# kevinh-e/BetaOne

Measured on AMD Instinct MI355X. Metric: mcts_nodes_per_sec, higher is better.
Workload: dtype f32 (3 x f16 split, f32 accumulate)

## Files before the change

betaone_amd/csrc/bo_chess.h:

```cpp
#pragma once
#include "bo_wave.h"

#define BO_MAX_MOVES 256
#define BO_NUM_ACTIONS 4672

enum { BB_P = 0, BB_N = 1, BB_B = 2, BB_R = 3, BB_Q = 4, BB_K = 5, BB_WHITE = 6, BB_BLACK = 7 };

struct DPos {
    uint64_t bb[8];
    uint32_t flags;
    int32_t halfmove;
    int32_t fullmove;
    uint32_t khash;
};
#define F_TURN 0x1u
#define F_CASTLE_SHIFT 1
#define F_CASTLE_MASK 0x1Eu
#define F_EP_SHIFT 8
#define F_EP_MASK (0x7Fu << 8)
#define F_IRREV 0x8000u
#define F_EPKEY_SHIFT 16
#define F_EPKEY_MASK (0x7Fu << 16)
#define F_KEY_MASK (F_TURN | F_CASTLE_MASK | F_EPKEY_MASK)

// ... 358 lines not shown
    o = bC + ((i1 >> 16) & 255) - cC;
    for (uint64_t t = tC; t;) {
        int to = bo_msb64(t);
        t ^= BIT(to);
        if (BIT(to) & promo_rank) { out[o++] = MV(s, to, 5); out[o++] = MV(s, to, 4); out[o++] = MV(s, to, 3); out[o++] = MV(s, to, 2); }
        else out[o++] = MV(s, to, 0);
    }
    o = b1 + ((i1 >> 24) & 255) - c1;
    if (t1) {
        int to = bo_lsb64(t1);
        if (t1 & promo_rank) { out[o++] = MV(s, to, 5); out[o++] = MV(s, to, 4); out[o++] = MV(s, to, 3); out[o++] = MV(s, to, 2); }
        else out[o++] = MV(s, to, 0);
    }
    if (t2) out[b2 + (i2 & 255) - c2] = MV(s, bo_lsb64(t2), 0);
    if (epc) out[bF + ((i2 >> 8) & 255) - cF] = MV(s, pos_ep(P), 0);
    bo_sync();
    *in_check_out = nchk > 0;
    return total;
}
BO_DEV_NOINLINE int bo_movegen(const DPos &P, bo_mv *out, bool *in_check_out) { return bo_movegen_inline(P, out, in_check_out); }
```

betaone_amd/csrc/bo_engine.cpp:

```cpp
#include "../../include/betaone_engine.h"
#include "../../include/betaone_lab.h"

#include "bo_tree.h"
#include "bo_fastw.h"
#include "bo_select_wide.h"
#include "bo_replay.h"
#include "bo_train.h"
#include "bo_pgn.h"
#include "bo_san.h"
#include "bo_analyse.h"
#include "bo_perft.h"
#include "bo_nn_fused.h"
#include "bo_conv.h"
#include "bo_tower.h"
#include "bo_tower_wg.h"
#include "bo_tower_h.h"
#include "bo_tower_s.h"
#include "bo_tower_s16.h"
#include "bo_tower_h16.h"
#include "bo_heads.h"
#include "bo_tower_b1.h"
#include "bo_rt.h"
#include "bo_hostrng.h"

// ... 16 lines not shown
        int _rc = (call);                                                                            \
        if (_rc != 0) return fail(BO_E_HIP, std::string(#call) + ": " + rt_errstr(_rc));             \
    } while (0)

struct bo_engine {
    Eng d;
    FastW f;
    int fast_reuse = 1;
    int sel_profile = 0, sel_pending = 0;
    long long sel_launches = 0;
    double sel_ms = 0.0;
#if !defined(BO_WAVE_EMU)
    hipEvent_t sel_ev0 = nullptr, sel_ev1 = nullptr;
#endif
    bool fast = false;
    bo_config cfg;
    int device;
    std::vector<void *> allocs;
    int *d_go = nullptr, *d_action = nullptr;
    std::vector<int> h_i32;
    std::vector<HostRng> rng;
    int *d_res_blk = nullptr, *d_info_blk = nullptr;
    int *h_res = nullptr, *h_info = nullptr;
    int watch_seen = 0;
    double *h_noise = nullptr;
    int *h_go = nullptr;
    int *h_action = nullptr;
    int action_flip = 0;
    rt_event ev_action[2]{};
    bool ev_action_made[2] = {false, false};
// ... 157 lines not shown
    for (int k = 1; k <= cfg->mcts_batch_size; k++) {
        const double r = (double)(int)(cfg->widen_coeff * sqrt((double)k)) / (double)k;
        if (r > per_sim) per_sim = r;
    }
    c.NCAP = fast ? 2 : (int)ceil(c.S * per_sim) + 2 * root_m + 4;
    c.nstride = c.NCAP;
    c.PLY_CAP = cfg->max_plies; c.TRK_CAP = cfg->max_plies;
    c.UL_MAX = fast ? 1 : c.B; c.CH_MAX = ch_max < 1 ? 1 : ch_max;
    c.cpuct = (float)cfg->cpuct;
    c.keep = (float)(1.0 - cfg->dirichlet_epsilon);
    c.eps = cfg->dirichlet_epsilon;
    c.use_noise = cfg->dirichlet_alpha > 0 ? 1 : 0;
    c.root_m = root_m;
    c.profile = 0;
    { const char *v = getenv("BETAONE_BURST_TWO_PATHS"); c.burst_two = (v && v[0] == '0') ? 0 : 1; }
    c.root_q = 0;
    const size_t G = (size_t)c.G, N = G * (size_t)c.NCAP;
    Eng &d = e->d;
    int rc = 0;
    float *sq = nullptr, *rcp = nullptr; int *wl = nullptr;
    rc |= e->alloc(&sq, (size_t)c.S + 2); rc |= e->alloc(&wl, (size_t)c.B + 1); rc |= e->alloc(&rcp, (size_t)c.S + 3);
    int **iscal[] = {&d.sims_done, &d.n_nodes, &d.rows, &d.n_runs, &d.n_ul, &d.req_nlegal, &d.status,
                     &d.trk_n, &d.n_hist, &d.ctx_mode, &d.root_nch, &d.stat_evals,
                     &d.stat_flushes, &d.stat_term_sims, &d.stat_levels, &d.stat_children_scanned, &e->d_go, &e->d_action};
    for (int **p : iscal) rc |= e->alloc(p, G);
    const size_t res_ints = G * (4 + 2 * (size_t)BO_RES_CAP) + 4, info_ints = G * 18;
    rc |= e->alloc(&e->d_res_blk, res_ints); rc |= e->alloc(&e->d_info_blk, info_ints);
    if (!rc) {
        d.res_n = e->d_res_blk; d.res_best_idx = e->d_res_blk + G; d.res_best_mv = e->d_res_blk + 2 * G; d.res_total = e->d_res_blk + 3 * G;
        d.res_idx = e->d_res_blk + 4 * G; d.res_val = reinterpret_cast<float *>(e->d_res_blk + 4 * G + G * BO_RES_CAP);
        d.res_watch = e->d_res_blk + G * (4 + 2 * (size_t)BO_RES_CAP); d.watch = nullptr; d.watch_n = 1;
        d.phase = e->d_info_blk; d.req_node = e->d_info_blk + G; d.root_nlegal = e->d_info_blk + 2 * G; d.root_term = e->d_info_blk + 3 * G;
        d.ply = e->d_info_blk + 4 * G;
        e->d_turn_action = e->d_info_blk + 5 * G; e->d_turn_state = e->d_info_blk + 6 * G; e->d_turn_cres = e->d_info_blk + 7 * G;
        e->d_turn_rv = reinterpret_cast<float *>(e->d_info_blk + 15 * G); e->d_turn_resigned = e->d_info_blk + 16 * G;
        e->d_turn_rnext = e->d_info_blk + 17 * G;
        rt_memset(e->d_res_blk, 0, res_ints * 4, nullptr); rt_memset(e->d_info_blk, 0, info_ints * 4, nullptr);
    }
    rc |= rt_host_alloc((void **)&e->h_res, res_ints * 4); rc |= rt_host_alloc((void **)&e->h_info, info_ints * 4);
    rc |= rt_host_alloc((void **)&e->h_noise, G * BO_MAX_MOVES * sizeof(double)); rc |= rt_host_alloc((void **)&e->h_go, G * 4);
    rc |= rt_host_alloc((void **)&e->h_action, 2 * G * 4);
    rc |= rt_host_alloc((void **)&e->h_turn_u, G * sizeof(double)); rc |= rt_host_alloc((void **)&e->h_turn_flags, G * 4);
    rc |= e->alloc(&e->d_turn_pw, (size_t)cfg->num_simulations + 1);
    { const char *v = getenv("BETAONE_TURN_COPIES"); e->ship = !(v && v[0] == '1'); }
    rc |= e->alloc(&d.gpos, G * c.PLY_CAP); rc |= e->alloc(&d.trk, G * c.TRK_CAP); rc |= e->alloc(&d.trk_cnt, G * c.TRK_CAP);
    rc |= e->alloc(&d.hist, G * 7);
    rc |= e->alloc(&d.n_visits, N); rc |= e->alloc(&d.parent, N); rc |= e->alloc(&d.first_child, N); rc |= e->alloc(&d.n_children, N);
    rc |= e->alloc(&d.q, N); rc |= e->alloc(&d.prior, N); rc |= e->alloc(&d.move, N); rc |= e->alloc(&d.term, N);
    rc |= e->alloc(&d.eval_slot, N); rc |= e->alloc(&d.npos, N);
    rc |= e->alloc(&d.run_leaf, G * c.B); rc |= e->alloc(&d.run_cnt, G * c.B);
    rc |= e->alloc(&d.ul_node, G * c.UL_MAX); rc |= e->alloc(&d.ul_nlegal, G * c.UL_MAX); rc |= e->alloc(&d.ul_value, G * c.UL_MAX);
    rc |= e->alloc(&d.ul_move, G * c.UL_MAX * BO_CH_CAP); rc |= e->alloc(&d.ul_prior, G * c.UL_MAX * BO_CH_CAP);
    rc |= e->alloc(&d.req_moves, G * BO_MAX_MOVES); rc |= e->alloc(&d.root_moves, G * BO_MAX_MOVES);
    rc |= e->alloc(&d.root_child_rank, G * 2 * BO_CH_CAP); rc |= e->alloc(&d.noise, G * BO_MAX_MOVES);
    rc |= e->alloc(&d.played, G * c.PLY_CAP);
    rc |= e->alloc(&d.prof, G * BO_PROF_SLOTS);
    rc |= e->alloc(&d.resign_cnt, 2 * G); rc |= e->alloc(&e->d_root_value, G);
    if (!rc) rt_memset(d.resign_cnt, 0, 2 * G * 4, nullptr);
    d.played_now = nullptr;
    if (fast) {
        FastW &f = e->f;
        const size_t L = (size_t)cfg->leaves_per_step;
        f.L = (int)L;
        f.sel_ut = 2; f.sel_flags = FW_SEL_OCT;
        const size_t expansions = (size_t)c.S + L + 2;
        f.NG = cfg->fast_arena_granules > 0 ? cfg->fast_arena_granules : (int)((6 * expansions + 8) * (32 / BO_FW_GR));
        if (f.NG < 64 || f.NG > BO_FW_LINK_MASK) { bo_engine_destroy(e); return fail(BO_E_ARG, "fast_arena_granules out of range (64 .. 2^24 - 1)"); }
        const size_t NR = (size_t)f.NG * BO_FW_GR;
        rc |= e->alloc(&f.arena, G * 2 * NR); rc |= e->alloc(&f.amove, G * 2 * NR);
        f.CS = (FWC_HEAD + FWR_FIELDS * (int)L + 31) / 32 * 32;
        rc |= e->alloc(&f.ctl, G * (size_t)f.CS);
// ... 248 lines not shown
            if (e->sel_pending) {
                float ms = 0.0f;
                RT((int)hipEventSynchronize(e->sel_ev1));
                RT((int)hipEventElapsedTime(&ms, e->sel_ev0, e->sel_ev1));
                e->sel_ms += ms; e->sel_launches++; e->sel_pending = 0;
            }
            RT((int)hipEventRecord(e->sel_ev0, (hipStream_t)stream));
        }
#endif
        RT(launch_fw_select(e, value_dev, policy_kind, stream));
#if !defined(BO_WAVE_EMU)
        if (e->sel_profile) { RT((int)hipEventRecord(e->sel_ev1, (hipStream_t)stream)); e->sel_pending = 1; }
#endif
        RT(RT_LAUNCH(bo_k_fw_leaf, rows, stream, e->d, e->f, nn_in_dev));
    } else {
        RT(RT_LAUNCH(bo_k_step, e->d.c.G, stream, e->d, policy_dev, value_dev, policy_kind, nn_in_dev, vt));
    }
    return BO_OK;
}
extern "C" int bo_step(bo_engine *e, const float *policy_dev, const float *value_dev, int policy_kind, float *nn_in_dev,
                       void *stream) {
    if (!e || !nn_in_dev) return fail(BO_E_ARG, "null argument");
    if (policy_kind != BO_POLICY_NONE && (!policy_dev || !value_dev)) return fail(BO_E_ARG, "policy/value required");
    return step_launch(e, policy_dev, value_dev, policy_kind, nn_in_dev, stream, StepTail{nullptr, nullptr, nullptr, nullptr, 0});
}
extern "C" int bo_step_heads(bo_engine *e, const float *logits_dev, const float *vpart_dev, const float *b1_dev, const float *w2_dev,
                             const float *b2_dev, int rows, float *nn_in_dev, void *stream) {
    if (!e || !nn_in_dev || !logits_dev || !vpart_dev || !b1_dev || !w2_dev || !b2_dev) return fail(BO_E_ARG, "null argument");
    if (e->fast) return fail(BO_E_CONFIG, "bo_step_heads: the reference-semantics search only (fast mode evaluates rows, not games)");
    if (rows < e->d.c.G) return fail(BO_E_ARG, "bo_step_heads: the partial sums must hold a row per game (rows >= G)");
    return step_launch(e, logits_dev, nullptr, BO_POLICY_LOGITS, nn_in_dev, stream, StepTail{vpart_dev, b1_dev, w2_dev, b2_dev, rows});
// ... 2185 lines not shown
```

betaone_amd/csrc/bo_rt.h:

```cpp
#pragma once
#include <stddef.h>
#include <stdlib.h>
#include <string.h>

#if defined(BO_WAVE_EMU)
static inline int rt_set_device(int) { return 0; }
static inline int rt_malloc(void **p, size_t n) { *p = malloc(n ? n : 1); if (*p) memset(*p, 0xCD, n); return *p ? 0 : -1; }
static inline void rt_free(void *p) { free(p); }
static inline int rt_h2d(void *d, const void *h, size_t n, void *) { memcpy(d, h, n); return 0; }
static inline int rt_d2h(void *h, const void *d, size_t n, void *) { memcpy(h, d, n); return 0; }
static inline int rt_memset(void *d, int v, size_t n, void *) { memset(d, v, n); return 0; }
static inline int rt_sync(void *) { return 0; }
static inline int rt_host_alloc(void **p, size_t n) { *p = calloc(n ? n : 1, 1); return *p ? 0 : -1; }
static inline void rt_host_free(void *p) { free(p); }
static inline int rt_h2d_2d(void *d, size_t dpitch, const void *h, size_t hpitch, size_t width, size_t height, void *) {
    for (size_t r = 0; r < height; r++) memcpy((char *)d + r * dpitch, (const char *)h + r * hpitch, width);
    return 0;
}
static inline int rt_d2h_2d(void *h, size_t hpitch, const void *d, size_t dpitch, size_t width, size_t height, void *) {
    for (size_t r = 0; r < height; r++) memcpy((char *)h + r * hpitch, (const char *)d + r * dpitch, width);
    return 0;
}
typedef int rt_event;
static inline int rt_event_create(rt_event *) { return 0; }
static inline int rt_event_record(rt_event, void *) { return 0; }
static inline int rt_event_sync(rt_event) { return 0; }
static inline void rt_event_destroy(rt_event) {}
static inline const char *rt_errstr(int) { return "emulator error"; }
#define RT_LAUNCH(kernel, grid, stream, ...) (bo_emu::launch((grid), [&]() { kernel(__VA_ARGS__); }), 0)
#else
#include <hip/hip_runtime.h>
static inline int rt_set_device(int d) { return (int)hipSetDevice(d); }
static inline int rt_malloc(void **p, size_t n) { return (int)hipMalloc(p, n ? n : 1); }
static inline void rt_free(void *p) { (void)hipFree(p); }
static inline int rt_h2d(void *d, const void *h, size_t n, void *s) { return (int)hipMemcpyAsync(d, h, n, hipMemcpyHostToDevice, (hipStream_t)s); }
static inline int rt_d2h(void *h, const void *d, size_t n, void *s) { return (int)hipMemcpyAsync(h, d, n, hipMemcpyDeviceToHost, (hipStream_t)s); }
static inline int rt_memset(void *d, int v, size_t n, void *s) { return (int)hipMemsetAsync(d, v, n, (hipStream_t)s); }
static inline int rt_sync(void *s) { return (int)hipStreamSynchronize((hipStream_t)s); }
static inline int rt_host_alloc(void **p, size_t n) { return (int)hipHostMalloc(p, n ? n : 1, hipHostMallocDefault); }
static inline void rt_host_free(void *p) { (void)hipHostFree(p); }
static inline int rt_h2d_2d(void *d, size_t dpitch, const void *h, size_t hpitch, size_t width, size_t height, void *s) {
    return (int)hipMemcpy2DAsync(d, dpitch, h, hpitch, width, height, hipMemcpyHostToDevice, (hipStream_t)s);
}
static inline int rt_d2h_2d(void *h, size_t hpitch, const void *d, size_t dpitch, size_t width, size_t height, void *s) {
    return (int)hipMemcpy2DAsync(h, hpitch, d, dpitch, width, height, hipMemcpyDeviceToHost, (hipStream_t)s);
}
typedef hipEvent_t rt_event;
static inline int rt_event_create(rt_event *ev) { return (int)hipEventCreateWithFlags(ev, hipEventDisableTiming); }
static inline int rt_event_record(rt_event ev, void *s) { return (int)hipEventRecord(ev, (hipStream_t)s); }
static inline int rt_event_sync(rt_event ev) { return (int)hipEventSynchronize(ev); }
static inline void rt_event_destroy(rt_event ev) { (void)hipEventDestroy(ev); }
static inline const char *rt_errstr(int e) { return hipGetErrorString((hipError_t)e); }
#define RT_LAUNCH(kernel, grid, stream, ...)                                                                   \
    ([&]() -> int {                                                                                            \
        hipLaunchKernelGGL(kernel, dim3((unsigned)(grid)), dim3(64), 0, (hipStream_t)(stream), __VA_ARGS__);   \
        return (int)hipGetLastError();                                                                         \
    }())
#endif
```

betaone_amd/csrc/bo_tree.h:

```cpp
#pragma once
#include "bo_chess.h"
#include <math.h>

#define BO_CH_CAP 32
#define BO_PATH_CAP 1024
#define BO_RES_CAP 256
#define BO_PLANES 120
#ifndef BO_PROF_SLOTS
#define BO_PROF_SLOTS 16
#endif
#define BO_ROW (BO_PLANES * 64)

enum { PH_IDLE = 0, PH_RUN = 1, PH_DONE = 2 };
enum { ST_OK = 0, ST_NODE_OVERFLOW = 1, ST_DEPTH_OVERFLOW = 2, ST_NAN_SCORE = 4, ST_PLY_OVERFLOW = 8,
       ST_ILLEGAL_ACTION = 16, ST_UL_OVERFLOW = 32, ST_TRK_OVERFLOW = 64 };
enum { POLICY_NONE = 0, POLICY_LOGITS = 1, POLICY_PROBS = 2 };

struct EngCfg {
    int G, S, B;
    int NCAP, PLY_CAP, TRK_CAP;
    int nstride;
    int UL_MAX, CH_MAX;
    float cpuct, keep;
    double eps;
    int use_noise;
    int root_m;
    int profile;
    int burst_two;
    int root_q;
};

struct Eng {
    EngCfg c;
    const float *sqrt_lut;
    const float *rcp_lut;
    const int *widen_lut;
    int *phase, *sims_done, *n_nodes, *rows, *n_runs, *n_ul, *req_node, *req_nlegal, *status;
    int *ply, *trk_n, *n_hist, *ctx_mode, *root_nlegal, *root_term, *root_nch;
    int *stat_evals, *stat_flushes, *stat_term_sims, *stat_levels, *stat_children_scanned;
    DPos *gpos, *trk, *hist;
    int *trk_cnt;
    int *n_visits, *parent, *first_child, *n_children;
    float *q, *prior;
// ... 4 lines not shown
    int *run_leaf, *run_cnt;
    int *ul_node, *ul_nlegal;
    float *ul_value;
    bo_mv *ul_move;
    float *ul_prior;
    bo_mv *req_moves, *root_moves;
    int *root_child_rank;
    double *noise;
    bo_mv *played;
    int *res_n, *res_idx, *res_best_idx, *res_best_mv, *res_total;
    float *res_val;
    int watch_n;
    int *watch, *res_watch;
    int *played_now;
    int *resign_cnt;
    unsigned long long *prof;
};

#define NOFF(e, g) ((size_t)(g) * (size_t)(e).c.nstride)

BO_DEV float bo_expf(float x) {
#if defined(BO_WAVE_EMU)
    return expf(x);
#else
    return __expf(x);
#endif
}
struct bo_f4 { float x, y, z, w; };
BO_DEV float bo_exp_row(float x) { return expf(x); }
#if defined(BO_WAVE_EMU)
// ... 84 lines not shown
        const int node = in ? path[j] : 0;
        const uint32_t fl = in ? e.npos[no + node].flags : 0u;
        const uint32_t kh = in ? e.npos[no + node].khash : 0u;
        const uint64_t irr = bo_ballot(in && j >= 1 && (fl & F_IRREV));
        const uint64_t below = BIT(lane) - 1;
        const bool take = in && j < d && (irr & below) == 0;
        const uint64_t tk = bo_ballot(take);
        if (take) {
            const int o = cnt + bo_popc64(tk & below);
            if (o < BO_CHAIN_CAP) { cb.hash[o] = kh; cb.ref[o] = node; }
        }
        cnt += bo_popc64(tk);
        stop = irr != 0;
    }
    if (!stop) cnt = chain_collect_history(e, g, cb, cnt);
    bo_sync();
    return cnt;
}

template <class PosFn, class CollectFn>
BO_DEV int terminal_eval_with(const Eng &e, int g, PosFn tree_pos, const DPos &P, const bo_mv *mv, int n, bool in_check, bo_mv *scratch,
                              ChainBuf &cb, CollectFn collect) {
    if (n == 0 && in_check) return 1;
    if (insufficient_material(P)) return 2;
    if (n == 0) return 2;
    if (P.halfmove >= 150) return 2;
    const int npred = collect();
    const int nn = npred < BO_CHAIN_CAP ? npred : BO_CHAIN_CAP;
    int same = 0;
    for (int i = bo_lane(); i < nn; i += 64)
        if (cb.hash[i] == P.khash && key_equal(chain_entry(e, g, tree_pos, cb.ref[i]), P)) same++;
// ... 72 lines not shown
BO_DEV void encode_static(const Eng &e, int g, float *row) {
    const int s = bo_lane();
    const int nh = e.n_hist[g];
    const DPos *h = e.hist + (size_t)g * 7;
    for (int pl = 0; pl < (7 - nh) * 14; pl++) row[pl * 64 + s] = 0.0f;
    for (int i = 0; i < nh; i++) {
        DPos H = h[i];
        encode_block(row, 7 - nh + i, H, tracker_reps(e, g, H));
    }
}
BO_DEV void encode_leaf(const Eng &e, int g, float *row, const DPos &P) {
    encode_block(row, 7, P, tracker_reps(e, g, P));
    encode_scalars(row, P);
}

BO_DEV int select_leaf(const Eng &e, int g, int *flags, int *path, int *depth_out, const float *lut) {
    const size_t no = NOFF(e, g);
    const int lane = bo_lane();
    int cur = 0, levels = 0, scanned = 0;
    if (lane == 0) path[0] = 0;
    int nc = e.n_children[no], fc = e.first_child[no];
    int pv = e.n_visits[no], pv_next = pv;
    for (;;) {
        if (nc == 0) break;
        const float sp = lut[pv];
        float score = -__builtin_inff();
        int n = 0, c_fc = 0, c_nc = 0;
        if (lane < nc) {
            n = e.n_visits[no + fc + lane];
            c_fc = e.first_child[no + fc + lane];
            c_nc = e.n_children[no + fc + lane];
// ... 28 lines not shown
        score = __builtin_bit_cast(float, bo_readlane(__builtin_bit_cast(int, score), 0));
        bi = bo_readlane(bi, 0);
        if (!(score > -__builtin_inff())) { *flags |= ST_NAN_SCORE; bi = 0; }
        cur = fc + bi;
        levels++;
        if (lane == 0) path[levels] = cur;
        scanned += nc;
        pv = pv_next;
        pv_next = bo_readlane(n, bi);
        fc = bo_readlane(c_fc, bi);
        nc = bo_readlane(c_nc, bi);
        if (levels >= BO_PATH_CAP - 1) { *flags |= ST_DEPTH_OVERFLOW; break; }
    }
    if (lane == 0) { e.stat_levels[g] += levels; e.stat_children_scanned[g] += scanned; }
    *depth_out = levels;
    bo_sync();
    return cur;
}

#define BO_BURST_LEVELS 4
#define BO_BURST_FITS(S) (2 * (S) + 5 <= BO_NUM_ACTIONS)
BO_DEV_NOINLINE float bo_div_general(float x, float fn) { return x / fn; }
BO_DEV float bo_div_count(float x, float fn, float y) {
    const float q0 = x * y;
    const float r = __builtin_fmaf(-fn, q0, x);
    float q = __builtin_fmaf(r, y, q0);
    const float a = q0 < 0.0f ? -q0 : q0;
    if (x == 0.0f) q = q0;
    else if (!(a >= 1e-30f && a <= 1e30f)) q = bo_div_general(x, fn);
    return q;
}
// ... 35 lines not shown
    int b_cn = 0, b_cterm = -1;
    float b_cq = 0.0f, b_cp = 0.0f;
    bool b_have = false;
    if (two) {
        b_have = grp >= c && grp < db && j < b_nc;
        b_cn = b_have ? e.n_visits[no + b_fc + j] : 0;
        b_cq = b_have ? e.q[no + b_fc + j] : 0.0f;
        b_cp = b_have ? e.prior[no + b_fc + j] : 0.0f;
        b_cterm = (b_have && grp == db - 1 && e.n_children[no + b_fc + j] == 0) ? (int)e.term[no + b_fc + j] : -1;
    }
    float v_cur = v, v_oth = vb;
    int d_oth = db;
    int done = 0;
    const int S = e.c.S;
    if (!*staged) {
        bo_sync();
        for (int t = lane; t < 2 * S + 5; t += 64) lds[t] = t < S + 2 ? e.sqrt_lut[t] : e.rcp_lut[t - (S + 2)];
        bo_sync();
        *staged = true;
    }
#define BO_SQ(i) lds[(i) <= S + 1 ? (i) : S + 1]
#define BO_RC(i) lds[S + 2 + ((i) <= S + 2 ? (i) : S + 2)]
    int pvl = nv[0];
#pragma unroll
    for (int k = 1; k < BO_BURST_LEVELS; k++)
        if (grp == k) pvl = nv[k - 1];
    float t1 = e.c.cpuct * cp, b_t1 = e.c.cpuct * b_cp;
    float y1 = BO_RC(1 + cn);
    float b_y1 = BO_RC(1 + b_cn);
    uint64_t last_bits = d > 0 ? (0xFFFFull << (16 * (d - 1))) : 0ull;
    bool last_l = last;
    int pv = pvl;
    const bool root_q = e.c.root_q != 0;
// ... 97 lines not shown
            { int o = BO_ROW_XCHG(bterm, 1); bterm = o > bterm ? o : bterm; }
            { int o = BO_ROW_XCHG(bterm, 2); bterm = o > bterm ? o : bterm; }
            { int o = BO_ROW_XCHG(bterm, 3); bterm = o > bterm ? o : bterm; }
            const int src = 16 * (d - 1);
            const int nb = bo_readlane(bi, src), nt = bo_readlane(bterm, src);
            if (!(nt > 0)) break;
            if (last_l) my_chosen = nb;
            v_cur = nt == 1 ? 1.0f : 0.0f;
        }
    }
#undef BO_SQ
#undef BO_RC
    if (have) { e.n_visits[no + my_fc + j] = cn; e.q[no + my_fc + j] = cq; }
    if (two && b_have) { e.n_visits[no + b_fc + j] = b_cn; e.q[no + b_fc + j] = b_cq; }
    if (lane == 0) { e.n_visits[no] = nv[0]; if (root_q) e.q[no] = rq; }
    bo_sync();
    return done;
}

BO_DEV void backup_run(const Eng &e, int g, int leaf, float v, int cnt, int *scratch, int *flags, const int *known = nullptr,
                       int known_depth = -1) {
    const size_t no = NOFF(e, g);
    int d = 0;
    if (known_depth >= 0) {
        d = known_depth + 1;
    } else {
        for (int x = leaf; x >= 0 && d < BO_PATH_CAP; x = e.parent[no + x]) {
            if (bo_lane() == 0) scratch[d] = x;
            d++;
        }
        bo_sync();
    }
    for (int i = bo_lane(); i < d; i += 64) {
        const int nd = known_depth >= 0 ? known[known_depth - i] : scratch[i];
        const float val = (i & 1) ? -v : v;
        int n = e.n_visits[no + nd];
        float qv = e.q[no + nd];
        for (int c = 0; c < cnt; c++) {
            n += 1;
            const float dd = val - qv;
            const float ee = dd / (float)n;
            qv = qv + ee;
        }
        e.n_visits[no + nd] = n;
        e.q[no + nd] = qv;
    }
    bo_sync();
}

BO_DEV void init_node(const Eng &e, size_t no, int idx, int par, float prior, bo_mv m, const DPos &P) {
    e.n_visits[no + idx] = 0;
    e.q[no + idx] = 0.0f;
    e.prior[no + idx] = prior;
    e.parent[no + idx] = par;
    e.first_child[no + idx] = 0;
    e.n_children[no + idx] = 0;
    e.move[no + idx] = m;
    e.term[no + idx] = -1;
    e.eval_slot[no + idx] = -1;
    e.npos[no + idx] = P;
}

// ... 9 lines not shown
        int k = 0;
        for (int r = 0; r < n_runs; r++) k += rl[r] == leaf ? rc[r] : 0;
        int c = e.widen_lut[k];
        const int nl = e.ul_nlegal[uo];
        if (c <= 0 || c > nl) c = nl;
        if (c > e.c.CH_MAX) c = e.c.CH_MAX;
        if (n_nodes + c > e.c.NCAP) { *flags |= ST_NODE_OVERFLOW; c = e.c.NCAP - n_nodes; }
        if (lane < c) {
            const DPos P = e.npos[no + leaf];
            const bo_mv m = e.ul_move[uo * BO_CH_CAP + lane];
            init_node(e, no, n_nodes + lane, leaf, e.ul_prior[uo * BO_CH_CAP + lane], m, make_move(P, m));
        }
        if (lane == 0) { e.first_child[no + leaf] = n_nodes; e.n_children[no + leaf] = c; }
        n_nodes += c;
    }
    bo_sync();
    for (int r = 0; r < n_runs; r++) {
        const int leaf = rl[r];
        const int slot = e.eval_slot[no + leaf];
        const bool known = leaf == cur_leaf && cur_depth >= 0;
        backup_run(e, g, leaf, e.ul_value[(size_t)g * e.c.UL_MAX + slot], rc[r], path, flags, known ? cur_path : nullptr, known ? cur_depth : -1);
    }
    *n_nodes_io = n_nodes;
    if (lane == 0) e.stat_flushes[g] += 1;
}

BO_DEV float np_sum_4672(const float *a) {
    const int L = bo_lane();
    const float *b = a + (L >> 3) * 584 + (L & 7) * 72;
    const int n = (L & 7) == 7 ? 80 : 72;
    float r0 = b[0], r1 = b[1], r2 = b[2], r3 = b[3], r4 = b[4], r5 = b[5], r6 = b[6], r7 = b[7];
// ... 30 lines not shown
    if (kind == POLICY_PROBS) {
        for (int i = lane; i < BO_NUM_ACTIONS; i += 64) out[i] = row[i];
    } else {
        float mx, sum;
        bo_f4 v[BO_ROW_IT];
        row_load_max_sum(row, v, &mx, &sum);
        BO_UNROLL
        for (int i = 0; i < BO_ROW_IT; i++) {
            const int k = lane + 64 * i;
            if (k < BO_ROW_N4) {
                out[4 * k] = bo_exp_row(v[i].x - mx) / sum; out[4 * k + 1] = bo_exp_row(v[i].y - mx) / sum;
                out[4 * k + 2] = bo_exp_row(v[i].z - mx) / sum; out[4 * k + 3] = bo_exp_row(v[i].w - mx) / sum;
            }
        }
    }
    bo_sync();
}

BO_DEV void apply_root(const Eng &e, int g, const float *row, int kind, StepShared &sh, int *n_nodes_io, int *flags) {
    const size_t no = NOFF(e, g);
    const int lane = bo_lane();
    const int n = e.root_nlegal[g];
    const bo_mv *mv = e.root_moves + (size_t)g * BO_MAX_MOVES;
    load_probs(row, kind, sh.probs);
    int m = e.c.root_m < n ? e.c.root_m : n;
    if (m > BO_CH_CAP) m = BO_CH_CAP;
    for (int j = lane; j < n; j += 64) sh.pv[j] = sh.probs[move_to_index(mv[j])];
    if (lane < 2 * BO_CH_CAP) sh.rank_of[lane] = -1;
    bo_sync();
    for (int j = lane; j < n; j += 64) {
        int r = stable_rank(sh.pv, n, j);
        if (r < m) sh.rank_of[r] = j;
    }
    bo_sync();
    const DPos P = e.npos[no];
    int nch = m;
    if (lane < m) {
        int j = sh.rank_of[lane];
        init_node(e, no, 1 + lane, 0, sh.pv[j], mv[j], make_move(P, mv[j]));
        e.root_child_rank[(size_t)g * 2 * BO_CH_CAP + lane] = j;
    }
    bo_sync();
    if (e.c.use_noise) {
        const double *nz = e.noise + (size_t)g * BO_MAX_MOVES;
        for (int j = lane; j < n; j += 64) {
            const int idx = move_to_index(mv[j]);
            const float a = e.c.keep * sh.probs[idx];
            const double s2 = (double)a + e.c.eps * nz[j];
            sh.probs[idx] = (float)s2;
        }
        bo_sync();
        const float sum = np_sum_4672(sh.probs);
        const float denom = sum + 1e-12f;
        for (int j = lane; j < n; j += 64) sh.pv[j] = sh.probs[move_to_index(mv[j])] / denom;
        bo_sync();
    }
    for (int j = lane; j < n; j += 64) {
        int r = stable_rank(sh.pv, n, j);
        if (r < m) sh.rank_of[BO_CH_CAP + r] = j;
    }
    bo_sync();
    for (int r = 0; r < m; r++) {
        const int j = sh.rank_of[BO_CH_CAP + r];
        bool present = false;
        for (int k = 0; k < m; k++) present = present || sh.rank_of[k] == j;
        if (!present) {
            if (lane == 0) {
                init_node(e, no, 1 + nch, 0, sh.pv[j], mv[j], make_move(P, mv[j]));
                e.root_child_rank[(size_t)g * 2 * BO_CH_CAP + nch] = j;
            }
            nch++;
        }
    }
    if (lane == 0) { e.first_child[no] = 1; e.n_children[no] = nch; e.root_nch[g] = nch; }
    *n_nodes_io = 1 + nch;
    bo_sync();
}

struct StepTail { const float *vpart, *b1, *w2, *b2; int rows; };
struct TailRegs { float part[4][16], b1[4], w2[4], b2; };
BO_DEV void tail_load(const StepTail &t, int g, TailRegs &r) {
    const int lane = bo_lane();
    BO_UNROLL
    for (int w = 0; w < 4; w++) {
        BO_UNROLL
        for (int ks = 0; ks < 16; ks++) r.part[w][ks] = t.vpart[((size_t)ks * t.rows + g) * 256 + lane + 64 * w];
        r.b1[w] = t.b1[lane + 64 * w];
        r.w2[w] = t.w2[lane + 64 * w];
    }
    r.b2 = t.b2[0];
}
// ... 2 lines not shown
    BO_UNROLL
    for (int w = 0; w < 4; w++) {
        float h = 0.0f;
        BO_UNROLL
        for (int ks = 0; ks < 16; ks++) h += r.part[w][ks];
        h += r.b1[w];
        s[w] = (h > 0.0f ? h : 0.0f) * r.w2[w];
    }
    for (int m = 32; m >= 1; m >>= 1) {
        BO_UNROLL
        for (int w = 0; w < 4; w++) s[w] = s[w] + bo_shfl_xor_f(s[w], m);
    }
    return tanhf(((s[0] + s[1]) + (s[2] + s[3])) + r.b2);
}

BO_DEV void apply_leaf(const Eng &e, int g, int leaf, const float *row, int kind, const float *value_of, const StepTail &vt, StepShared &sh,
                       int *n_ul_io, int *flags) {
    const size_t no = NOFF(e, g);
    const int lane = bo_lane();
    const int n = e.req_nlegal[g];
    const bo_mv *mv = e.req_moves + (size_t)g * BO_MAX_MOVES;
    int slot = *n_ul_io;
    if (slot >= e.c.UL_MAX) { *flags |= ST_UL_OVERFLOW; slot = e.c.UL_MAX - 1; }
    const size_t uo = (size_t)g * e.c.UL_MAX + slot;
    float value;
    if (kind == POLICY_PROBS) {
        value = value_of[g];
        for (int j = lane; j < n; j += 64) sh.pv[j] = row[move_to_index(mv[j])];
    } else {
        float mx, sum;
        if (vt.vpart) {
            TailRegs tr;
            tail_load(vt, g, tr);
            row_max_sum(row, &mx, &sum);
            value = tail_value(tr);
        } else {
            value = value_of[g];
            row_max_sum(row, &mx, &sum);
        }
        for (int j = lane; j < n; j += 64) sh.pv[j] = bo_exp_row(row[move_to_index(mv[j])] - mx) / sum;
    }
    bo_sync();
    const int M = n < e.c.CH_MAX ? n : e.c.CH_MAX;
    for (int j = lane; j < n; j += 64) {
        int r = stable_rank(sh.pv, n, j);
        if (r < M) { e.ul_move[uo * BO_CH_CAP + r] = mv[j]; e.ul_prior[uo * BO_CH_CAP + r] = sh.pv[j]; }
    }
    if (lane == 0) {
        e.ul_node[uo] = leaf;
        e.ul_nlegal[uo] = n;
        e.ul_value[uo] = value;
        e.eval_slot[no + leaf] = (short)slot;
    }
    *n_ul_io = slot + 1;
    bo_sync();
}


BO_DEV int step_body(const Eng &e, int g, const float *policy, const float *value, int kind, float *nn_in, StepShared &sh, const StepTail &vt) {
    const int lane = bo_lane();
    const size_t no = NOFF(e, g);
    int flags = 0;
    int sims = e.sims_done[g], rows = e.rows[g], n_runs = e.n_runs[g], n_ul = e.n_ul[g], n_nodes = e.n_nodes[g];
    int req = e.req_node[g];
    int *rl = e.run_leaf + (size_t)g * e.c.B, *rc = e.run_cnt + (size_t)g * e.c.B;
    float *row = nn_in + (size_t)g * BO_ROW;

    const bool prof = e.c.profile != 0;
    unsigned long long pc[8] = {0, 0, 0, 0, 0, 0, 0, 0};
    int n_iter = 0, n_first = 0, n_burst = 0, n_burst_sims = 0, n_general = 0, n_swaps = 0;
    unsigned long long tk = prof ? bo_clock() : 0ull;
    const unsigned long long t_start = tk;
#define BO_PROF(slot)                                                    \
    if (prof) { const unsigned long long _n = bo_clock(); pc[slot] += _n - tk; tk = _n; }
    if (req >= 0 && kind == POLICY_NONE) return n_nodes;
    const float *lut = e.sqrt_lut;
    if (req >= 0) {
        if (req == 0) apply_root(e, g, policy + (size_t)g * BO_NUM_ACTIONS, kind, sh, &n_nodes, &flags);
        else apply_leaf(e, g, req, policy + (size_t)g * BO_NUM_ACTIONS, kind, value, vt, sh, &n_ul, &flags);
        req = -1;
    }
    BO_PROF(0)
    int phase = PH_RUN;
    bool burst_tables_staged = false;
    int term_budget = e.c.B;
    int b_depth = 0;
    float b_tv = 0.0f;
    int path_leaf = -1, path_depth = -1;
    for (;;) {
        if (sims >= e.c.S) {
            if (rows > 0) { flush_pending(e, g, n_runs, n_ul, &n_nodes, sh.path2, &flags, path_leaf, sh.path, path_depth); rows = n_runs = n_ul = 0; }
            BO_PROF(5)
            phase = PH_DONE;
            break;
        }
        int depth;
        const int leaf = select_leaf(e, g, &flags, sh.path, &depth, lut);
        path_leaf = leaf; path_depth = depth;
        n_iter++;
        BO_PROF(1)
        int t = e.term[no + leaf];
        if (t < 0) {
            n_first++;
            const DPos P = e.npos[no + leaf];
            bool chk;
            const int n = bo_movegen(P, sh.moves, &chk);
            t = terminal_eval(e, g, sh.path, depth, P, sh.moves, n, chk, sh.moves2, sh.chain);
            if (lane == 0) e.term[no + leaf] = (signed char)t;
            if (t == 0) {
                for (int j = lane; j < n; j += 64) e.req_moves[(size_t)g * BO_MAX_MOVES + j] = sh.moves[j];
                if (lane == 0) e.req_nlegal[g] = n;
            }
            bo_sync();
            BO_PROF(2)
        }
        if (t > 0) {
            const float tv = t == 1 ? 1.0f : 0.0f;
            int applied = 1;
            bool small = depth <= BO_BURST_LEVELS && BO_BURST_FITS(e.c.S);
            for (int k = 0; k < depth && small; k++) small = e.n_children[no + sh.path[k]] <= 16;
            BO_PROF(6)
            const int may = e.c.S - sims < term_budget ? e.c.S - sims : term_budget;
            if (small) {
                const bool small_b = b_depth > 0 && e.c.burst_two != 0;
                applied = terminal_burst(e, g, sh.path, depth, tv, may, sh.probs, &burst_tables_staged, sh.bpath, small_b ? b_depth : 0, b_tv, &n_swaps);
                n_burst++; n_burst_sims += applied;
                bo_sync();
                if (lane <= depth) sh.bpath[lane] = sh.path[lane];
                b_depth = depth; b_tv = tv;
                bo_sync();
            }
            else { backup_run(e, g, leaf, tv, 1, sh.path2, &flags, sh.path, depth); n_general++; }
            BO_PROF(7)
            sims += applied;
            term_budget -= applied;
            if (lane == 0) e.stat_term_sims[g] += applied;
            BO_PROF(3)
            if (term_budget <= 0 && sims < e.c.S) break;
            continue;
        }
        if (e.eval_slot[no + leaf] < 0) {
            encode_leaf(e, g, row, e.npos[no + leaf]);
            req = leaf;
            if (lane == 0) e.stat_evals[g] += 1;
            BO_PROF(4)
            break;
        }
        int cnt = e.c.B - rows;
        if (cnt > e.c.S - sims) cnt = e.c.S - sims;
        if (lane == 0) { rl[n_runs] = leaf; rc[n_runs] = cnt; }
        n_runs++;
        rows += cnt;
        sims += cnt;
        bo_sync();
        if (rows >= e.c.B) { flush_pending(e, g, n_runs, n_ul, &n_nodes, sh.path2, &flags, path_leaf, sh.path, path_depth); rows = n_runs = n_ul = 0; }
        BO_PROF(5)
    }
#undef BO_PROF
    if (prof && lane == 0) {
        const unsigned long long total = bo_clock() - t_start;
        if (e.c.profile == 1 || total > (unsigned long long)e.c.profile) {
            unsigned long long *pp = e.prof + (size_t)g * BO_PROF_SLOTS;
            pp[10] += (unsigned long long)n_burst; pp[11] += (unsigned long long)n_burst_sims; pp[12] += (unsigned long long)n_general;
            pp[13] += pc[6]; pp[14] += pc[7]; pp[15] += (unsigned long long)n_swaps;
            for (int i = 0; i < 6; i++) pp[i] += pc[i];
            pp[6] += total;
            pp[7] += 1;
            pp[8] += (unsigned long long)n_iter;
            pp[9] += (unsigned long long)n_first;
        }
    }
    if (lane == 0) {
        e.sims_done[g] = sims; e.rows[g] = rows; e.n_runs[g] = n_runs; e.n_ul[g] = n_ul; e.n_nodes[g] = n_nodes;
        e.req_node[g] = req; e.phase[g] = phase;
        if (flags) e.status[g] |= flags;
    }
    return n_nodes;
}
BO_KERNEL void bo_k_step(Eng e, const float *policy, const float *value, int kind, float *nn_in, StepTail vt) {
    BO_SHARED StepShared sh;
    const int g = bo_block();
    if (e.phase[g] != PH_RUN) return;
    step_body(e, g, policy, value, kind, nn_in, sh, vt);
}

BO_DEV int root_prepare(const Eng &e, int g, StepShared &sh) {
    const size_t no = NOFF(e, g);
    const int lane = bo_lane();
    const int ply = e.ply[g];
    const DPos P = e.gpos[(size_t)g * e.c.PLY_CAP + ply];
    if (lane == 0) {
        init_node(e, no, 0, -1, 1.0f, 0, P);
        e.n_nodes[g] = 1; e.sims_done[g] = 0; e.rows[g] = 0; e.n_runs[g] = 0; e.n_ul[g] = 0;
        e.req_node[g] = -1; e.phase[g] = PH_IDLE; e.root_nch[g] = 0;
        if (e.ctx_mode[g] == 0) {
            int nh = ply < 7 ? ply : 7;
            e.n_hist[g] = nh;
            for (int i = 0; i < nh; i++) e.hist[(size_t)g * 7 + i] = e.gpos[(size_t)g * e.c.PLY_CAP + ply - nh + i];
        }
// ... 330 lines not shown
```

betaone_amd/csrc/bo_wave.h:

```cpp
#pragma once
#include <stdint.h>

#if defined(BO_WAVE_EMU)
#include "wave_emu.h"
#else
#include <hip/hip_runtime.h>
#define BO_DEV __device__ __forceinline__
#define BO_DEV_NOINLINE __device__ __noinline__
#define BO_KERNEL extern "C" __global__ __launch_bounds__(64)
#define BO_SHARED __shared__
#define BO_CONST_TABLE __device__ const

BO_DEV int bo_lane() { return (int)(threadIdx.x & 63u); }
BO_DEV int bo_block() { return (int)blockIdx.x; }
BO_DEV uint64_t bo_ballot(bool p) { return __ballot(p); }
BO_DEV void bo_sync() { __syncthreads(); }
BO_DEV int bo_shfl(int v, int src) { return __shfl(v, src, 64); }
BO_DEV int bo_shfl_xor(int v, int m) { return __shfl_xor(v, m, 64); }
BO_DEV int bo_shfl_up(int v, int d) { return __shfl_up(v, d, 64); }
BO_DEV int bo_atomic_add(int *p, int v) { return atomicAdd(p, v); }
BO_DEV int bo_atomic_or(int *p, int v) { return atomicOr(p, v); }
BO_DEV uint64_t bo_bitrev64(uint64_t x) { return __builtin_bitreverse64(x); }
BO_DEV unsigned long long bo_clock() { return (unsigned long long)clock64(); }
#define BO_ROW_XCHG(v, kind) \
// ... 10 lines not shown
    const int src = kind == 0 ? (l ^ 1) : kind == 1 ? (l ^ 2) : kind == 2 ? ((l & ~7) | (7 - (l & 7))) : ((l & ~15) | (15 - (l & 15)));
    return bo_shfl(v, src);
}
#define BO_ROW_XCHG(v, kind) bo_row_xchg_emu((v), (kind))
#endif

#if defined(BO_WAVE_EMU)
BO_DEV void bo_wave_sync() { bo_emu::rendezvous(); }
#else
BO_DEV void bo_wave_sync() {
    __builtin_amdgcn_fence(__ATOMIC_ACQ_REL, "wavefront");
    __builtin_amdgcn_wave_barrier();
}
#endif

BO_DEV float bo_shfl_f(float v, int src) { return __builtin_bit_cast(float, bo_shfl(__builtin_bit_cast(int, v), src)); }
BO_DEV float bo_shfl_xor_f(float v, int m) { return __builtin_bit_cast(float, bo_shfl_xor(__builtin_bit_cast(int, v), m)); }
BO_DEV uint64_t bo_shfl_u64(uint64_t v, int src) {
    uint32_t lo = (uint32_t)bo_shfl((int)(uint32_t)v, src), hi = (uint32_t)bo_shfl((int)(uint32_t)(v >> 32), src);
    return ((uint64_t)hi << 32) | lo;
}
BO_DEV int bo_popc64(uint64_t x) { return __builtin_popcountll(x); }
BO_DEV int bo_msb64(uint64_t x) { return 63 - __builtin_clzll(x); }
BO_DEV int bo_lsb64(uint64_t x) { return __builtin_ctzll(x); }

BO_DEV int bo_wave_sum(int v) {
    for (int m = 1; m < 64; m <<= 1) v += bo_shfl_xor(v, m);
    return v;
}
BO_DEV int bo_wave_scan_desc(int v) {
// ... 16 lines not shown
```

Baseline: 74.93 million.

## Use wave-level sync, cache selection path, split tail kernel, add packed step launch

Replaces workgroup barriers with wavefront-scoped fences and barriers throughout the step kernel, since each game runs in a single wave. It persists the selected leaf's path, depth and flags per game so the next step can skip re-selecting the same leaf after its evaluation returns. The value-tail variant becomes a separate templated kernel, removing a runtime branch. It also adds an optional 4-games-per-workgroup launch behind an environment variable. The kept-path shortcut assumes the tree has not changed between the request and its result, and the added s_waitcnt(0) may stall on outstanding memory operations.

```diff
diff --git a/betaone_amd/csrc/bo_chess.h b/betaone_amd/csrc/bo_chess.h
--- a/betaone_amd/csrc/bo_chess.h
+++ b/betaone_amd/csrc/bo_chess.h
@@ -396,7 +396,7 @@
     }
     if (t2) out[b2 + (i2 & 255) - c2] = MV(s, bo_lsb64(t2), 0);
     if (epc) out[bF + ((i2 >> 8) & 255) - cF] = MV(s, pos_ep(P), 0);
-    bo_sync();
+    bo_wsync();
     *in_check_out = nchk > 0;
     return total;
 }
diff --git a/betaone_amd/csrc/bo_engine.cpp b/betaone_amd/csrc/bo_engine.cpp
--- a/betaone_amd/csrc/bo_engine.cpp
+++ b/betaone_amd/csrc/bo_engine.cpp
@@ -54,6 +54,7 @@
     hipEvent_t sel_ev0 = nullptr, sel_ev1 = nullptr;
 #endif
     bool fast = false;
+    bool step_pack4 = false;
     bo_config cfg;
     int device;
     std::vector<void *> allocs;
@@ -241,6 +242,7 @@
     c.root_m = root_m;
     c.profile = 0;
     { const char *v = getenv("BETAONE_BURST_TWO_PATHS"); c.burst_two = (v && v[0] == '0') ? 0 : 1; }
+    { const char *v = getenv("BETAONE_STEP_KEEP_PATH"); c.keep_path = (v && v[0] == '0') ? 0 : 1; }
     c.root_q = 0;
     const size_t G = (size_t)c.G, N = G * (size_t)c.NCAP;
     Eng &d = e->d;
@@ -270,6 +272,7 @@
     rc |= rt_host_alloc((void **)&e->h_turn_u, G * sizeof(double)); rc |= rt_host_alloc((void **)&e->h_turn_flags, G * 4);
     rc |= e->alloc(&e->d_turn_pw, (size_t)cfg->num_simulations + 1);
     { const char *v = getenv("BETAONE_TURN_COPIES"); e->ship = !(v && v[0] == '1'); }
+    { const char *v = getenv("BETAONE_STEP_PACK"); e->step_pack4 = v && v[0] == '4' && v[1] == 0; }
     rc |= e->alloc(&d.gpos, G * c.PLY_CAP); rc |= e->alloc(&d.trk, G * c.TRK_CAP); rc |= e->alloc(&d.trk_cnt, G * c.TRK_CAP);
     rc |= e->alloc(&d.hist, G * 7);
     rc |= e->alloc(&d.n_visits, N); rc |= e->alloc(&d.parent, N); rc |= e->alloc(&d.first_child, N); rc |= e->alloc(&d.n_children, N);
@@ -282,6 +285,8 @@
     rc |= e->alloc(&d.root_child_rank, G * 2 * BO_CH_CAP); rc |= e->alloc(&d.noise, G * BO_MAX_MOVES);
     rc |= e->alloc(&d.played, G * c.PLY_CAP);
     rc |= e->alloc(&d.prof, G * BO_PROF_SLOTS);
+    rc |= e->alloc(&d.spath, G * BO_SPATH_INTS);
+    if (!rc) rt_memset(d.spath, 0xFF, G * BO_SPATH_INTS * 4, nullptr);
     rc |= e->alloc(&d.resign_cnt, 2 * G); rc |= e->alloc(&e->d_root_value, G);
     if (!rc) rt_memset(d.resign_cnt, 0, 2 * G * 4, nullptr);
     d.played_now = nullptr;
@@ -560,7 +565,17 @@
 #endif
         RT(RT_LAUNCH(bo_k_fw_leaf, rows, stream, e->d, e->f, nn_in_dev));
     } else {
-        RT(RT_LAUNCH(bo_k_step, e->d.c.G, stream, e->d, policy_dev, value_dev, policy_kind, nn_in_dev, vt));
+        const int G = e->d.c.G;
+#if RT_HAS_WIDE_LAUNCH
+        if (e->step_pack4) {
+            const int wgs = (G + BO_STEP_PACK - 1) / BO_STEP_PACK;
+            if (vt.vpart) RT(RT_LAUNCH_WAVES(bo_k_step4_tail, wgs, BO_STEP_PACK, stream, e->d, policy_dev, policy_kind, nn_in_dev, vt));
+            else RT(RT_LAUNCH_WAVES(bo_k_step4, wgs, BO_STEP_PACK, stream, e->d, policy_dev, value_dev, policy_kind, nn_in_dev));
+            return BO_OK;
+        }
+#endif
+        if (vt.vpart) RT(RT_LAUNCH(bo_k_step_tail, G, stream, e->d, policy_dev, policy_kind, nn_in_dev, vt));
+        else RT(RT_LAUNCH(bo_k_step, G, stream, e->d, policy_dev, value_dev, policy_kind, nn_in_dev));
     }
     return BO_OK;
 }
diff --git a/betaone_amd/csrc/bo_rt.h b/betaone_amd/csrc/bo_rt.h
--- a/betaone_amd/csrc/bo_rt.h
+++ b/betaone_amd/csrc/bo_rt.h
@@ -28,6 +28,7 @@
 static inline void rt_event_destroy(rt_event) {}
 static inline const char *rt_errstr(int) { return "emulator error"; }
 #define RT_LAUNCH(kernel, grid, stream, ...) (bo_emu::launch((grid), [&]() { kernel(__VA_ARGS__); }), 0)
+#define RT_HAS_WIDE_LAUNCH 0
 #else
 #include <hip/hip_runtime.h>
 static inline int rt_set_device(int d) { return (int)hipSetDevice(d); }
@@ -56,4 +57,10 @@
         hipLaunchKernelGGL(kernel, dim3((unsigned)(grid)), dim3(64), 0, (hipStream_t)(stream), __VA_ARGS__);   \
         return (int)hipGetLastError();                                                                         \
     }())
+#define RT_HAS_WIDE_LAUNCH 1
+#define RT_LAUNCH_WAVES(kernel, grid, waves, stream, ...)                                                      \
+    ([&]() -> int {                                                                                            \
+        hipLaunchKernelGGL(kernel, dim3((unsigned)(grid)), dim3(64u * (waves)), 0, (hipStream_t)(stream), __VA_ARGS__); \
+        return (int)hipGetLastError();                                                                         \
+    }())
 #endif
diff --git a/betaone_amd/csrc/bo_tree.h b/betaone_amd/csrc/bo_tree.h
--- a/betaone_amd/csrc/bo_tree.h
+++ b/betaone_amd/csrc/bo_tree.h
@@ -5,6 +5,7 @@
 #define BO_CH_CAP 32
 #define BO_PATH_CAP 1024
 #define BO_RES_CAP 256
+#define BO_SPATH_INTS 64
 #define BO_PLANES 120
 #ifndef BO_PROF_SLOTS
 #define BO_PROF_SLOTS 16
@@ -27,6 +28,7 @@
     int root_m;
     int profile;
     int burst_two;
+    int keep_path;
     int root_q;
 };
 
@@ -61,6 +63,7 @@
     int *watch, *res_watch;
     int *played_now;
     int *resign_cnt;
+    int *spath;
     unsigned long long *prof;
 };
 
@@ -175,7 +178,7 @@
         stop = irr != 0;
     }
     if (!stop) cnt = chain_collect_history(e, g, cb, cnt);
-    bo_sync();
+    bo_wsync();
     return cnt;
 }
 
@@ -278,7 +281,7 @@
     encode_scalars(row, P);
 }
 
-BO_DEV int select_leaf(const Eng &e, int g, int *flags, int *path, int *depth_out, const float *lut) {
+BO_DEV int select_leaf(const Eng &e, int g, int *flags, int *path, int *depth_out, const float *lut, int *scanned_out) {
     const size_t no = NOFF(e, g);
     const int lane = bo_lane();
     int cur = 0, levels = 0, scanned = 0;
@@ -337,7 +340,8 @@
     }
     if (lane == 0) { e.stat_levels[g] += levels; e.stat_children_scanned[g] += scanned; }
     *depth_out = levels;
-    bo_sync();
+    *scanned_out = scanned;
+    bo_wsync();
     return cur;
 }
 
@@ -403,9 +407,9 @@
     int done = 0;
     const int S = e.c.S;
     if (!*staged) {
-        bo_sync();
+        bo_wsync();
         for (int t = lane; t < 2 * S + 5; t += 64) lds[t] = t < S + 2 ? e.sqrt_lut[t] : e.rcp_lut[t - (S + 2)];
-        bo_sync();
+        bo_wsync();
         *staged = true;
     }
 #define BO_SQ(i) lds[(i) <= S + 1 ? (i) : S + 1]
@@ -533,7 +537,7 @@
     if (have) { e.n_visits[no + my_fc + j] = cn; e.q[no + my_fc + j] = cq; }
     if (two && b_have) { e.n_visits[no + b_fc + j] = b_cn; e.q[no + b_fc + j] = b_cq; }
     if (lane == 0) { e.n_visits[no] = nv[0]; if (root_q) e.q[no] = rq; }
-    bo_sync();
+    bo_wsync();
     return done;
 }
 
@@ -548,7 +552,7 @@
             if (bo_lane() == 0) scratch[d] = x;
             d++;
         }
-        bo_sync();
+        bo_wsync();
     }
     for (int i = bo_lane(); i < d; i += 64) {
         const int nd = known_depth >= 0 ? known[known_depth - i] : scratch[i];
@@ -564,7 +568,7 @@
         e.n_visits[no + nd] = n;
         e.q[no + nd] = qv;
     }
-    bo_sync();
+    bo_wsync();
 }
 
 BO_DEV void init_node(const Eng &e, size_t no, int idx, int par, float prior, bo_mv m, const DPos &P) {
@@ -604,7 +608,7 @@
         if (lane == 0) { e.first_child[no + leaf] = n_nodes; e.n_children[no + leaf] = c; }
         n_nodes += c;
     }
-    bo_sync();
+    bo_wsync();
     for (int r = 0; r < n_runs; r++) {
         const int leaf = rl[r];
         const int slot = e.eval_slot[no + leaf];
@@ -665,7 +669,7 @@
             }
         }
     }
-    bo_sync();
+    bo_wsync();
 }
 
 BO_DEV void apply_root(const Eng &e, int g, const float *row, int kind, StepShared &sh, int *n_nodes_io, int *flags) {
@@ -678,12 +682,12 @@
     if (m > BO_CH_CAP) m = BO_CH_CAP;
     for (int j = lane; j < n; j += 64) sh.pv[j] = sh.probs[move_to_index(mv[j])];
     if (lane < 2 * BO_CH_CAP) sh.rank_of[lane] = -1;
-    bo_sync();
+    bo_wsync();
     for (int j = lane; j < n; j += 64) {
         int r = stable_rank(sh.pv, n, j);
         if (r < m) sh.rank_of[r] = j;
     }
-    bo_sync();
+    bo_wsync();
     const DPos P = e.npos[no];
     int nch = m;
     if (lane < m) {
@@ -691,7 +695,7 @@
         init_node(e, no, 1 + lane, 0, sh.pv[j], mv[j], make_move(P, mv[j]));
         e.root_child_rank[(size_t)g * 2 * BO_CH_CAP + lane] = j;
     }
-    bo_sync();
+    bo_wsync();
     if (e.c.use_noise) {
         const double *nz = e.noise + (size_t)g * BO_MAX_MOVES;
         for (int j = lane; j < n; j += 64) {
@@ -700,17 +704,17 @@
             const double s2 = (double)a + e.c.eps * nz[j];
             sh.probs[idx] = (float)s2;
         }
-        bo_sync();
+        bo_wsync();
         const float sum = np_sum_4672(sh.probs);
         const float denom = sum + 1e-12f;
         for (int j = lane; j < n; j += 64) sh.pv[j] = sh.probs[move_to_index(mv[j])] / denom;
-        bo_sync();
+        bo_wsync();
     }
     for (int j = lane; j < n; j += 64) {
         int r = stable_rank(sh.pv, n, j);
         if (r < m) sh.rank_of[BO_CH_CAP + r] = j;
     }
-    bo_sync();
+    bo_wsync();
     for (int r = 0; r < m; r++) {
         const int j = sh.rank_of[BO_CH_CAP + r];
         bool present = false;
@@ -725,7 +729,7 @@
     }
     if (lane == 0) { e.first_child[no] = 1; e.n_children[no] = nch; e.root_nch[g] = nch; }
     *n_nodes_io = 1 + nch;
-    bo_sync();
+    bo_wsync();
 }
 
 struct StepTail { const float *vpart, *b1, *w2, *b2; int rows; };
@@ -758,6 +762,7 @@
     return tanhf(((s[0] + s[1]) + (s[2] + s[3])) + r.b2);
 }
 
+template <bool TAIL>
 BO_DEV void apply_leaf(const Eng &e, int g, int leaf, const float *row, int kind, const float *value_of, const StepTail &vt, StepShared &sh,
                        int *n_ul_io, int *flags) {
     const size_t no = NOFF(e, g);
@@ -773,7 +778,7 @@
         for (int j = lane; j < n; j += 64) sh.pv[j] = row[move_to_index(mv[j])];
     } else {
         float mx, sum;
-        if (vt.vpart) {
+        if (TAIL) {
             TailRegs tr;
             tail_load(vt, g, tr);
             row_max_sum(row, &mx, &sum);
@@ -784,7 +789,7 @@
         }
         for (int j = lane; j < n; j += 64) sh.pv[j] = bo_exp_row(row[move_to_index(mv[j])] - mx) / sum;
     }
-    bo_sync();
+    bo_wsync();
     const int M = n < e.c.CH_MAX ? n : e.c.CH_MAX;
     for (int j = lane; j < n; j += 64) {
         int r = stable_rank(sh.pv, n, j);
@@ -797,10 +802,11 @@
         e.eval_slot[no + leaf] = (short)slot;
     }
     *n_ul_io = slot + 1;
-    bo_sync();
-}
-
-
+    bo_wsync();
+}
+
+
+template <bool TAIL>
 BO_DEV int step_body(const Eng &e, int g, const float *policy, const float *value, int kind, float *nn_in, StepShared &sh, const StepTail &vt) {
     const int lane = bo_lane();
     const size_t no = NOFF(e, g);
@@ -819,9 +825,18 @@
     if (prof) { const unsigned long long _n = bo_clock(); pc[slot] += _n - tk; tk = _n; }
     if (req >= 0 && kind == POLICY_NONE) return n_nodes;
     const float *lut = e.sqrt_lut;
+    int *spath = e.spath + (size_t)g * BO_SPATH_INTS;
+    int kept_leaf = -1, kept_depth = -1, kept_scanned = 0, kept_flags = 0, kept_node = 0;
     if (req >= 0) {
         if (req == 0) apply_root(e, g, policy + (size_t)g * BO_NUM_ACTIONS, kind, sh, &n_nodes, &flags);
-        else apply_leaf(e, g, req, policy + (size_t)g * BO_NUM_ACTIONS, kind, value, vt, sh, &n_ul, &flags);
+        else {
+            const int word = spath[lane];
+            apply_leaf<TAIL>(e, g, req, policy + (size_t)g * BO_NUM_ACTIONS, kind, value, vt, sh, &n_ul, &flags);
+            if (e.c.keep_path && bo_readlane(word, 0) == req) {
+                kept_leaf = req; kept_depth = bo_readlane(word, 1); kept_scanned = bo_readlane(word, 2); kept_flags = bo_readlane(word, 3);
+                kept_node = word;
+            }
+        }
         req = -1;
     }
     BO_PROF(0)
@@ -838,12 +853,21 @@
             phase = PH_DONE;
             break;
         }
-        int depth;
-        const int leaf = select_leaf(e, g, &flags, sh.path, &depth, lut);
+        int depth, leaf, scanned = 0;
+        const bool kept = kept_depth >= 0;
+        if (kept) {
+            leaf = kept_leaf; depth = kept_depth; scanned = kept_scanned; flags |= kept_flags;
+            if (lane >= 4 && lane - 4 <= depth) sh.path[lane - 4] = kept_node;
+            if (lane == 0) { e.stat_levels[g] += depth; e.stat_children_scanned[g] += scanned; }
+            kept_depth = -1;
+            bo_wsync();
+        } else {
+            leaf = select_leaf(e, g, &flags, sh.path, &depth, lut, &scanned);
+        }
         path_leaf = leaf; path_depth = depth;
         n_iter++;
         BO_PROF(1)
-        int t = e.term[no + leaf];
+        int t = kept ? 0 : e.term[no + leaf];
         if (t < 0) {
             n_first++;
             const DPos P = e.npos[no + leaf];
@@ -855,7 +879,7 @@
                 for (int j = lane; j < n; j += 64) e.req_moves[(size_t)g * BO_MAX_MOVES + j] = sh.moves[j];
                 if (lane == 0) e.req_nlegal[g] = n;
             }
-            bo_sync();
+            bo_wsync();
             BO_PROF(2)
         }
         if (t > 0) {
@@ -869,10 +893,10 @@
                 const bool small_b = b_depth > 0 && e.c.burst_two != 0;
                 applied = terminal_burst(e, g, sh.path, depth, tv, may, sh.probs, &burst_tables_staged, sh.bpath, small_b ? b_depth : 0, b_tv, &n_swaps);
                 n_burst++; n_burst_sims += applied;
-                bo_sync();
+                bo_wsync();
                 if (lane <= depth) sh.bpath[lane] = sh.path[lane];
                 b_depth = depth; b_tv = tv;
-                bo_sync();
+                bo_wsync();
             }
             else { backup_run(e, g, leaf, tv, 1, sh.path2, &flags, sh.path, depth); n_general++; }
             BO_PROF(7)
@@ -883,9 +907,15 @@
             if (term_budget <= 0 && sims < e.c.S) break;
             continue;
         }
-        if (e.eval_slot[no + leaf] < 0) {
+        if (!kept && e.eval_slot[no + leaf] < 0) {
             encode_leaf(e, g, row, e.npos[no + leaf]);
             req = leaf;
+            {
+                const bool fits = depth <= BO_SPATH_INTS - 5;
+                int word = lane == 0 ? leaf : lane == 1 ? (fits ? depth : -1) : lane == 2 ? scanned : flags;
+                if (lane >= 4 && fits && lane - 4 <= depth) word = sh.path[lane - 4];
+                spath[lane] = word;
+            }
             if (lane == 0) e.stat_evals[g] += 1;
             BO_PROF(4)
             break;
@@ -896,7 +926,7 @@
         n_runs++;
         rows += cnt;
         sims += cnt;
-        bo_sync();
+        bo_wsync();
         if (rows >= e.c.B) { flush_pending(e, g, n_runs, n_ul, &n_nodes, sh.path2, &flags, path_leaf, sh.path, path_depth); rows = n_runs = n_ul = 0; }
         BO_PROF(5)
     }
@@ -921,12 +951,36 @@
     }
     return n_nodes;
 }
-BO_KERNEL void bo_k_step(Eng e, const float *policy, const float *value, int kind, float *nn_in, StepTail vt) {
+BO_KERNEL void bo_k_step(Eng e, const float *policy, const float *value, int kind, float *nn_in) {
     BO_SHARED StepShared sh;
     const int g = bo_block();
     if (e.phase[g] != PH_RUN) return;
-    step_body(e, g, policy, value, kind, nn_in, sh, vt);
-}
+    step_body<false>(e, g, policy, value, kind, nn_in, sh, StepTail{nullptr, nullptr, nullptr, nullptr, 0});
+}
+BO_KERNEL void bo_k_step_tail(Eng e, const float *policy, int kind, float *nn_in, StepTail vt) {
+    BO_SHARED StepShared sh;
+    const int g = bo_block();
+    if (e.phase[g] != PH_RUN) return;
+    step_body<true>(e, g, policy, nullptr, kind, nn_in, sh, vt);
+}
+#if !defined(BO_WAVE_EMU)
+#define BO_STEP_PACK 4
+template <bool TAIL>
+BO_DEV void step_packed(const Eng &e, const float *policy, const float *value, int kind, float *nn_in, const StepTail &vt) {
+    BO_SHARED StepShared sh[BO_STEP_PACK];
+    const int w = bo_uniform((int)(threadIdx.x >> 6));
+    const int g = bo_block() * BO_STEP_PACK + w;
+    if (g >= e.c.G) return;
+    if (e.phase[g] != PH_RUN) return;
+    step_body<TAIL>(e, g, policy, value, kind, nn_in, sh[w], vt);
+}
+BO_KERNEL_WAVES(BO_STEP_PACK) void bo_k_step4(Eng e, const float *policy, const float *value, int kind, float *nn_in) {
+    step_packed<false>(e, policy, value, kind, nn_in, StepTail{nullptr, nullptr, nullptr, nullptr, 0});
+}
+BO_KERNEL_WAVES(BO_STEP_PACK) void bo_k_step4_tail(Eng e, const float *policy, int kind, float *nn_in, StepTail vt) {
+    step_packed<true>(e, policy, nullptr, kind, nn_in, vt);
+}
+#endif
 
 BO_DEV int root_prepare(const Eng &e, int g, StepShared &sh) {
     const size_t no = NOFF(e, g);
diff --git a/betaone_amd/csrc/bo_wave.h b/betaone_amd/csrc/bo_wave.h
--- a/betaone_amd/csrc/bo_wave.h
+++ b/betaone_amd/csrc/bo_wave.h
@@ -8,6 +8,7 @@
 #define BO_DEV __device__ __forceinline__
 #define BO_DEV_NOINLINE __device__ __noinline__
 #define BO_KERNEL extern "C" __global__ __launch_bounds__(64)
+#define BO_KERNEL_WAVES(N) extern "C" __global__ __launch_bounds__(64 * (N))
 #define BO_SHARED __shared__
 #define BO_CONST_TABLE __device__ const
 
@@ -48,6 +49,17 @@
 }
 #endif
 
+#if defined(BO_WAVE_EMU)
+BO_DEV void bo_wsync() { bo_emu::rendezvous(); }
+#else
+BO_DEV void bo_wsync() {
+    __builtin_amdgcn_fence(__ATOMIC_RELEASE, "wavefront");
+    __builtin_amdgcn_s_waitcnt(0);
+    __builtin_amdgcn_wave_barrier();
+    __builtin_amdgcn_fence(__ATOMIC_ACQUIRE, "wavefront");
+}
+#endif
+
 BO_DEV float bo_shfl_f(float v, int src) { return __builtin_bit_cast(float, bo_shfl(__builtin_bit_cast(int, v), src)); }
 BO_DEV float bo_shfl_xor_f(float v, int m) { return __builtin_bit_cast(float, bo_shfl_xor(__builtin_bit_cast(int, v), m)); }
 BO_DEV uint64_t bo_shfl_u64(uint64_t v, int src) {
```

After: 75.42 million (median of 6 runs). Within noise of the previous version (+0.7%).
